# pvphan/camera-calibration

Hardware: AMD Instinct MI355X
Metric: LM iters/sec & residuals/sec, 10k-view checkerboard @1/2/4/8 GPU (higher is better)
Workload: dtype f64

## Files before the change

camera-calibration_amd/_native.py:

```python
import ctypes
import os
import sys

import numpy as np

_HERE = os.path.dirname(os.path.abspath(__file__))
LIB_PATH = os.environ.get("CALIB_LM_LIBRARY") or os.path.join(_HERE, "lib", "libcalib_lm.so")

MODEL_RADTAN, MODEL_FISHEYE = 0, 1
DTYPE_F64, DTYPE_F32 = 0, 1
E_INVALID, E_HIP, E_SINGULAR, E_STATE = -1, -2, -3, -4
TRACE_HEADER = 5
LM_FUSED, LM_TWO_KERNEL = 0, 1

_c_double_p = ctypes.POINTER(ctypes.c_double)
_c_int64_p = ctypes.POINTER(ctypes.c_int64)
_c_int_p = ctypes.POINTER(ctypes.c_int)
_h = ctypes.c_void_p

SIGNATURES = {
    "calib_version": (ctypes.c_int, []),
    "calib_last_error": (ctypes.c_char_p, []),
    "calib_device_count": (ctypes.c_int, [_c_int_p]),
    "calib_create": (ctypes.c_int, [ctypes.c_int, ctypes.c_int, ctypes.c_int, ctypes.POINTER(_h)]),
# ... 17 lines not shown
                                            _c_double_p, ctypes.c_int]),
    "calib_decompose_params": (ctypes.c_int, [ctypes.c_int, ctypes.c_int64, _c_double_p, _c_double_p, _c_double_p,
                                              _c_double_p, ctypes.c_int]),
    "calib_refine_awk": (ctypes.c_int, [_h, _c_double_p, _c_double_p, _c_double_p, ctypes.c_int, ctypes.c_double,
                                        ctypes.c_double, ctypes.c_double, ctypes.c_double, _c_double_p, _c_int_p,
                                        _c_double_p]),
    "calib_lm_begin": (ctypes.c_int, [_h, _c_double_p, ctypes.c_int, ctypes.c_double, ctypes.c_double,
                                      ctypes.c_double, ctypes.c_double]),
    "calib_lm_reduce_size": (ctypes.c_int, [_h, _c_int64_p]),
    "calib_lm_bind_reduce_buffer": (ctypes.c_int, [_h, ctypes.c_void_p]),
    "calib_lm_local": (ctypes.c_int, [_h]),
    "calib_lm_update": (ctypes.c_int, [_h]),
    "calib_lm_run": (ctypes.c_int, [_h, ctypes.c_int, ctypes.c_int]),
    "calib_lm_run_sharded": (ctypes.c_int, [_h, ctypes.c_int, ctypes.c_int]),
    "calib_lm_done": (ctypes.c_int, [_h, _c_int_p]),
    "calib_lm_peek_trace": (ctypes.c_int, [_h, ctypes.c_int, _c_double_p, _c_int_p]),
    "calib_lm_end": (ctypes.c_int, [_h, _c_double_p, _c_double_p, _c_int_p, _c_double_p]),
    "calib_distort_points": (ctypes.c_int, [ctypes.c_int, ctypes.c_int64, _c_double_p, _c_double_p, _c_double_p]),
    "calib_project_with_distortion": (ctypes.c_int, [ctypes.c_int, ctypes.c_int64, _c_double_p, _c_double_p,
                                                     _c_double_p, _c_double_p]),
    "calib_refine_homographies": (ctypes.c_int, [ctypes.c_int64, _c_int64_p, _c_double_p, _c_double_p, _c_double_p,
                                                 ctypes.c_int, ctypes.c_int]),
    "calib_refine_poses": (ctypes.c_int, [ctypes.c_int, ctypes.c_int64, _c_int64_p, _c_double_p, _c_double_p, _c_double_p,
                                          _c_double_p, ctypes.c_int, ctypes.c_double, ctypes.c_double, ctypes.c_double,
                                          ctypes.c_double, _c_double_p, _c_int_p, _c_int_p, ctypes.c_int]),
    "calib_homography_jacobian": (ctypes.c_int, [ctypes.c_int64, _c_double_p, _c_double_p, _c_double_p, ctypes.c_int]),
    "calib_estimate_homographies": (ctypes.c_int, [ctypes.c_int64, _c_int64_p, _c_double_p, _c_double_p, _c_double_p,
                                                   ctypes.c_int, ctypes.c_int]),
    "calib_compute_extrinsics": (ctypes.c_int, [ctypes.c_int64, _c_double_p, _c_double_p, _c_double_p, ctypes.c_int]),
    "calib_distortion_normal_equations": (ctypes.c_int, [ctypes.c_int, ctypes.c_int64, _c_int64_p, _c_double_p,
# ... 94 lines not shown
```

camera-calibration_amd/csrc/calib_lm.hip:

```cpp
#include "../../include/calib_lm.h"
#include "kernels.hpp"
#include "host_rows.hpp"
#include "launch_plan.hpp"

#include <hip/hip_runtime.h>
#include <hip/hip_ext.h>
#include <algorithm>
#include <atomic>
#include <cmath>
#include <cstdio>
#include <cstdlib>
#include <dlfcn.h>
#include <chrono>
#include <future>
#include <memory>
#include <mutex>
#include <thread>
#include <cstring>
#include <new>
#include <string>
#include <type_traits>
#include <vector>

using namespace calib;
// ... 103 lines not shown
    DevBuf<LMState> st, st_eval;
    double* red = nullptr;
    void* comm = nullptr;
    DevBuf<double> rccl_test;
    int comm_ranks = 0, comm_rank = 0;
    void* peer_mem = nullptr;
    std::vector<void*> peer_open;
    DevBuf<unsigned long long*> peer_slots;
    std::vector<unsigned long long*> peer_slot_host;
    DevBuf<int> peer_flags;
    int peer_world = 0, peer_rank = 0;
    unsigned peer_epoch = 0;
    double peer_timeout_s = 60.0;
    bool peer_connected = false;
    bool exchange_round = false;
    int* host_done = nullptr;
    int* host_done_dev = nullptr;
    bool lm_active = false;
    int lm_max_iters = 0;
    int rounds_enqueued = 0;

    bool cov_pending = false;
    std::vector<int64_t> ext_offsets;
    bool ext_offsets_on_device = false;
    DevBuf<int64_t> ext_offsets_dev;
    DevBuf<double> view_err, cov_css, cov_views, cov_cross;
    DevBuf<int> cov_flag;

    bool stage_ready = false;
    void* stage_pinned = nullptr;
// ... 203 lines not shown
StreamMap stream_map(const calib_handle_s* h) {
    StreamMap sm;
    sm.share = h->plan.stream_share;
    sm.n4 = h->uniform_n / 4;
    sm.nv = h->nv;
    return sm;
}
int num_records(const calib_handle_s* h) { return std::max(h->n_items, 1) + h->plan.stream_waves; }

template <int MODEL>
int launch_fused_stream(calib_handle_s* h, const LMState* st, int sel) {
    const LaunchPlan& p = h->plan;
    launch_kind(h, 2, fused_stream_kernel<MODEL>, dim3(p.fused_blocks), dim3(256), 0, (const double*)h->P[0].p, (const double*)h->P[1].p,
                reinterpret_cast<const double2*>(h->uv.p), reinterpret_cast<const double2*>(h->XY.p),
                reinterpret_cast<const double*>(h->Z.p), reinterpret_cast<const double*>(h->VC.p), h->uniform_n,
                h->nv, p.stream_share, (const uint32_t*)h->emit_tab.p, (const int32_t*)h->stream_ops.p, st, sel, h->G[0].p, h->G[1].p,
                h->bpart.p);
    h->n_bpart = p.fused_blocks;
    LAUNCHED(h, "fused_stream_kernel");
    return CALIB_OK;
}

int launch_fused(calib_handle_s* h, const LMState* st, int sel) {
    if (h->plan.fused == FusedForm::Stream)
        return h->model == CALIB_MODEL_RADTAN ? launch_fused_stream<kRadtan>(h, st, sel)
                                              : launch_fused_stream<kFisheye>(h, st, sel);
    if (h->dtype == CALIB_DTYPE_F64)
        return h->model == CALIB_MODEL_RADTAN ? launch_fused_t<kRadtan, double>(h, st, sel)
                                              : launch_fused_t<kFisheye, double>(h, st, sel);
    return h->model == CALIB_MODEL_RADTAN ? launch_fused_t<kRadtan, float>(h, st, sel)
                                          : launch_fused_t<kFisheye, float>(h, st, sel);
// ... 7 lines not shown
    for (int r = 0; r < kPeerInline; ++r) x.slot8[r] = r < (int)h->peer_slot_host.size() ? h->peer_slot_host[(size_t)r] : nullptr;
    x.fault = h->peer_flags.p;
    x.notify = h->host_done_dev;
    x.timeout_ticks = (unsigned long long)(h->peer_timeout_s * 1e8);
    x.epoch = ++h->peer_epoch;
    x.world = h->peer_world;
    x.rank = h->peer_rank;
    return x;
}

int launch_schur(calib_handle_s* h, const LMState* st) {
    const LaunchPlan& p = h->plan;
    dim3 grid(p.schur_blocks, 3);
    auto launch = [&](auto kernel) {
        hipLaunchKernelGGL(kernel, grid, dim3(kSchurBlock), 0, h->stream, h->G[0].p, h->G[1].p, st, view_items(h), h->nv,
                           stream_map(h), h->bpart.p, h->n_bpart, h->part.p);
    };
    auto pick = [&](auto Lc) {
        constexpr int LL = decltype(Lc)::value;
        if (p.stream()) { if (p.wide_heads) launch(schur_kernel<LL, true, true>); else launch(schur_kernel<LL, false, true>); }
        else { if (p.wide_heads) launch(schur_kernel<LL, true, false>); else launch(schur_kernel<LL, false, false>); }
    };
    if (h->L == 10) pick(std::integral_constant<int, 10>{}); else pick(std::integral_constant<int, 9>{});
    LAUNCHED(h, "schur_kernel");
    return CALIB_OK;
}

int launch_schur_reduce(calib_handle_s* h, const LMState* st, double* red) {
    const int VA = variantSize(h->L);
    if (h->nv > 0) {
        const int rc = launch_schur(h, st);
// ... 11 lines not shown

template <int L, typename T>
int launch_update_backsub_t(calib_handle_s* h) {
    const LaunchPlan& p = h->plan;
    UpdArgs<T> a;
    a.G0 = h->G[0].p; a.G1 = h->G[1].p;
    a.st_in = st_cur(h); a.st_out = st_next(h);
    a.red = h->red;
    a.view_item0 = view_items(h);
    a.view_ext = h->view_ext.p;
    a.nv = h->nv;
    a.sm = stream_map(h);
    a.P0 = h->P[0].p; a.P1 = h->P[1].p;
    a.trace = h->trace.p;
    a.VC = reinterpret_cast<T*>(h->VC.p);
    auto launch = [&](auto kernel, int threads, const char* name) -> int {
        hipLaunchKernelGGL(kernel, dim3(p.update_blocks), dim3(threads), 0, h->stream, a);
        LAUNCHED(h, name);
        return CALIB_OK;
    };
    if (p.update == UpdateForm::Small)
        return p.stream() ? launch(update_backsub_small_kernel<L, T, true>, kUpdThreads, "update_backsub_small_kernel")
                          : launch(update_backsub_small_kernel<L, T, false>, kUpdThreads, "update_backsub_small_kernel");
    if (p.update == UpdateForm::Lane)
        return p.stream() ? launch(update_backsub_lane_kernel<L, T, true>, kSchurThreads, "update_backsub_lane_kernel")
                          : launch(update_backsub_lane_kernel<L, T, false>, kSchurThreads, "update_backsub_lane_kernel");
    return p.stream() ? launch(update_backsub_kernel<L, T, true>, kSchurThreads, "update_backsub_kernel")
                      : launch(update_backsub_kernel<L, T, false>, kSchurThreads, "update_backsub_kernel");
}

// ... 512 lines not shown
    }
    if (h->host_done) {
        if (h->lm_active) SYNC_H(h);
        *h->host_done = 0;
        s.notify = h->host_done_dev;
    }
    s.cur = 1;
    s.fixed_mask = (int)h->fixed_mask;
    s.max_iters = max_iters;
    HIP_TRY(hipMemsetAsync(h->st.p, 0, 2 * sizeof(LMState), h->stream));
    HIP_TRY(hipMemcpyAsync(h->st.p, &s, sizeof(s), hipMemcpyHostToDevice, h->stream));
    SYNC_H(h);
    h->lm_active = true;
    h->lm_max_iters = max_iters;
    h->rounds_enqueued = 0;
    return CALIB_OK;
}

int calib_lm_local(calib_handle_t h) {
    CHECK_H(h);
    if (!h->lm_active) return fail(CALIB_E_STATE, "calib_lm_begin has not been called");
    LMState* st = st_cur(h);
    int rc = CALIB_OK;
    if (h->rounds_enqueued == 0) {
        rc = launch_view_setup_any(h, h->P[0].p, h->P[1].p, st, 1);
        if (rc) return rc;
    }
    if (h->lm_mode == CALIB_LM_FUSED) {
        rc = launch_fused(h, st, 1);
        if (rc) return rc;
// ... 2 lines not shown
    h->n_bpart = 0;
    for (const auto& c : h->chunks) {
        rc = launch_jacobian(h, h->P[0].p, h->P[1].p, st, 1, true, true, false, false, c.p0, c.p1);
        if (rc) return rc;
        rc = launch_gram(h, st, 1, c.item0, c.item1, c.p0);
        if (rc) return rc;
    }
    return launch_schur_reduce(h, st, h->red);
}

int calib_lm_update(calib_handle_t h) {
    CHECK_H(h);
    if (!h->lm_active) return fail(CALIB_E_STATE, "calib_lm_begin has not been called");
    const int rc = launch_update_backsub(h);
    h->rounds_enqueued += 1;
    return rc;
}

namespace {
int peer_fault_check(calib_handle_s* h) {
    if (!h->peer_connected) return CALIB_OK;
    int fault = 0;
    HIP_TRY(hipMemcpy(&fault, h->peer_flags.p, sizeof(int), hipMemcpyDeviceToHost));
    if (fault)
        return fail(CALIB_E_HIP, "peer exchange: a rank's contribution did not arrive before the deadline "
                                 "(the ranks no longer run in lockstep, or a peer died)");
    return CALIB_OK;
}
}

int calib_lm_done(calib_handle_t h, int* out_done) {
    CHECK_H(h);
    if (!h->lm_active || !out_done) return fail(CALIB_E_STATE, "no LM run active");
    LMState s;
    HIP_TRY(hipMemcpyAsync(&s, st_cur(h), sizeof(s), hipMemcpyDeviceToHost, h->stream));
    SYNC_H(h);
    *out_done = s.done;
    return peer_fault_check(h);
}

int calib_lm_peek_trace(calib_handle_t h, int iter, double* out_row, int* out_iters) {
    CHECK_H(h);
    if (!h->lm_active || !out_row || !out_iters) return fail(CALIB_E_STATE, "no LM run active");
    if (iter < 0 || iter >= h->lm_max_iters) return fail(CALIB_E_INVALID, "trace row out of range");
    LMState s;
    const size_t w = (size_t)(CALIB_TRACE_HEADER + h->L);
    HIP_TRY(hipMemcpyAsync(&s, st_cur(h), sizeof(s), hipMemcpyDeviceToHost, h->stream));
    HIP_TRY(hipMemcpyAsync(out_row, h->trace.p + (size_t)iter * w, w * 8, hipMemcpyDeviceToHost, h->stream));
    SYNC_H(h);
    *out_iters = s.iters;
    return CALIB_OK;
}

namespace {
int lm_run(calib_handle_t h, int rounds, int check_every, bool sharded);
}

int calib_lm_run(calib_handle_t h, int rounds, int check_every) { return lm_run(h, rounds, check_every, false); }

int calib_lm_run_sharded(calib_handle_t h, int rounds, int check_every) {
    if (h && !h->comm && !h->peer_connected)
        return fail(CALIB_E_STATE, "neither calib_peer_connect nor calib_rccl_init has been called");
    return lm_run(h, rounds, check_every, true);
}

namespace {
int lm_run(calib_handle_t h, int rounds, int check_every, bool sharded) {
    CHECK_H(h);
    if (!h->lm_active) return fail(CALIB_E_STATE, "calib_lm_begin has not been called");
    const bool peers = sharded && h->peer_connected;
    for (int i = 0; i < rounds; ++i) {
        h->exchange_round = peers;
        int rc = calib_lm_local(h);
        h->exchange_round = false;
        if (rc) return rc;
        if (sharded && !peers) {
            rc = calib_lm_allreduce(h);
            if (rc) return rc;
        }
        rc = calib_lm_update(h);
        if (rc) return rc;
        if (peers && h->host_done && *static_cast<volatile int*>(h->host_done) == 2)
            return fail(CALIB_E_HIP, "peer exchange: a rank's contribution did not arrive before the deadline "
                                     "(the ranks no longer run in lockstep, or a peer died); no further rounds are enqueued");
        if (check_every > 0 && !sharded && h->host_done) {
            if (*static_cast<volatile int*>(h->host_done)) break;
        } else if (check_every > 0 && (i + 1) % check_every == 0 && i + 1 < rounds) {
            int done = 0;
            rc = calib_lm_done(h, &done);
            if (rc) return rc;
            if (done) break;
        }
    }
    return CALIB_OK;
}
}

int calib_rccl_load(const char* librccl_path) {
    std::lock_guard<std::mutex> lock(g_rccl_mutex);
    if (g_rccl.lib) return CALIB_OK;
    if (!librccl_path) return fail(CALIB_E_INVALID, "librccl path is null");
    void* lib = dlopen(librccl_path, RTLD_NOW | RTLD_GLOBAL);
    if (!lib) return fail(CALIB_E_HIP, std::string("dlopen librccl: ") + dlerror());
    RcclApi a;
    a.lib = lib;
    a.getUniqueId = reinterpret_cast<decltype(a.getUniqueId)>(dlsym(lib, "ncclGetUniqueId"));
    a.commInitRank = reinterpret_cast<decltype(a.commInitRank)>(dlsym(lib, "ncclCommInitRank"));
    a.allReduce = reinterpret_cast<decltype(a.allReduce)>(dlsym(lib, "ncclAllReduce"));
// ... 861 lines not shown
```

camera-calibration_amd/csrc/kernels.hpp:

```cpp
#pragma once
#include "point_model.hpp"
#include <stdint.h>
#include <type_traits>

namespace calib {

constexpr int kTile = 256;
constexpr int kGramChunk = 512;
constexpr int kGramUnroll = 4;
constexpr int kGRows = 0;
constexpr int kGStride = 96;
__host__ __device__ __forceinline__ constexpr int gvSlot(int L, int j) { return j < 5 ? L + 1 + j : 16 + L + 2; }
__host__ __device__ __forceinline__ constexpr int gvOfSlot(int L, int slot) {
    const int m = slot >> 4, n = (slot & 15) - L;
    return (m == 0 && n >= 1 && n <= 5) ? n - 1 : ((m == 1 && n == 2) ? 5 : -1);
}
constexpr int kPartStride = 112;
constexpr int kMaxL = 10;

constexpr int kEmitZero = 256;
constexpr int kEmitTile = 264;
constexpr int kEmitTabSize = kGStride + kPartStride;
inline void buildEmitTable(int C, uint32_t* tab ) {
    const int L = C - 6;
// ... 49 lines not shown
    o.x = __builtin_bit_cast(float, __builtin_amdgcn_ds_bpermute(a, __builtin_bit_cast(int, v.x)));
    o.y = __builtin_bit_cast(float, __builtin_amdgcn_ds_bpermute(a, __builtin_bit_cast(int, v.y)));
    return o;
}

struct LMState {
    double lam, err_cur, last_err, lam_min, lam_max, err_min;
    int cur;
    int round;
    int iters;
    int max_iters;
    int done;
    int error;
    int accepted_last;
    int fixed_mask;
    int* notify;
    double dc[kMaxL];
    double B[kMaxL * kMaxL];
    double gc[kMaxL];
};

__host__ __device__ constexpr int variantSize(int L) { return 2 * L * L + 2 * L + 2; }
__host__ __device__ constexpr int reduceSize(int L) { return 2 * variantSize(L); }

__device__ __forceinline__ const double* selectP(const double* P0, const double* P1,
                                                 const LMState* st, int sel) {
    if (sel == 0) return P0;
    return (st->cur ^ 1) ? P1 : P0;
}

// ... 240 lines not shown

struct BlockAcc {
    double d0u = 0.0, d0v = 0.0, d1u = 0.0, d1v = 0.0, d2u = 0.0;
    int bi, bj, trow, tcol0, tcol1, tcol2;
    __device__ __forceinline__ explicit BlockAcc(int lane) {
        const int k = lane >> 4;
        bi = (lane >> 2) & 3; bj = lane & 3;
        trow = 4 * bi + k; tcol0 = 4 * bi + bj; tcol1 = 4 * ((bi + 1) & 3) + bj; tcol2 = 4 * ((bi + 2) & 3) + bj;
    }
    __device__ __forceinline__ void contract(const double2& ja, const double2& jb, double ha, double hc) {
        d0u = __builtin_amdgcn_mfma_f64_4x4x4f64(ja.x, ja.x, d0u, 0, 0, 0);
        d0v = __builtin_amdgcn_mfma_f64_4x4x4f64(ja.y, ja.y, d0v, 0, 0, 0);
        d1u = __builtin_amdgcn_mfma_f64_4x4x4f64(ja.x, jb.x, d1u, 0, 0, 0);
        d1v = __builtin_amdgcn_mfma_f64_4x4x4f64(ja.y, jb.y, d1v, 0, 0, 0);
        d2u = __builtin_amdgcn_mfma_f64_4x4x4f64(ha, hc, d2u, 0, 0, 0);
    }
    __device__ __forceinline__ void park(double* TU, double* TV) const {
        TU[trow * 16 + tcol0] = d0u;  TV[trow * 16 + tcol0] = d0v;
        TU[trow * 16 + tcol1] = d1u;  TV[trow * 16 + tcol1] = d1v;
        TU[tcol1 * 16 + trow] = d1u;  TV[tcol1 * 16 + trow] = d1v;
        double* T2nd = bi < 2 ? TU : TV;
        T2nd[trow * 16 + tcol2] = d2u;
        T2nd[tcol2 * 16 + trow] = d2u;
    }
};

template <int MODEL, typename T, bool G44, bool MULTI>
__global__ __launch_bounds__(64 * kFusedWaves, (sizeof(T) == 4 ? (MULTI ? 5 : 6)
                                                             : (ModelTraits<MODEL>::C == 16 ? 4 : 3))) void fused_kernel(const double* __restrict__ P0, const double* __restrict__ P1,
                                                    const typename Pair<T>::type* __restrict__ uv,
// ... 267 lines not shown
            const Src sv = locate(iv, true);
            put(sv.lane, sv.acc == 1 ? 7 : (sv.acc == 3 ? 9 : 10), 1, slot);
        }
    }
    return ok;
}

constexpr int kStreamMinBlocks = 4;
template <int MODEL>
__global__ __launch_bounds__(64 * kFusedWaves, kStreamMinBlocks) void fused_stream_kernel(const double* __restrict__ P0, const double* __restrict__ P1,
                                                              const double2* __restrict__ uv, const double2* __restrict__ XY,
                                                              const double* __restrict__ Z, const double* __restrict__ VC,
                                                              int n, int nv, int share,
                                                              const uint32_t* __restrict__ emit_tab,
                                                              const int32_t* __restrict__ stream_ops,
                                                              const LMState* __restrict__ st, int sel,
                                                              double* __restrict__ G0, double* __restrict__ G1,
                                                              double* __restrict__ part) {
    using T = double;
    using T2 = double2;
    constexpr int C = ModelTraits<MODEL>::C, L = C - 6;
    using Slab = FusedSlab<T, C>;
    constexpr int ROWS = Slab::ROWS, WAVES = Slab::WAVES, SLAB = Slab::SIZE;
    constexpr bool RCOL = Slab::RCOL, ONES = Slab::ONES;
    __shared__ __attribute__((aligned(16))) unsigned char smem[Slab::BYTES];
    __shared__ __attribute__((aligned(16))) double svc[WAVES][2 * kViewStride];
    __shared__ __attribute__((aligned(16))) int32_t sops[64 * kStreamOps];
    int fin = 0, useP1 = 0;
    auto readState = [&]() {
        if (sel) {
            fin = st->done;
            useP1 = st->cur ^ 1;
        }
    };
    const int lane = threadIdx.x & 63;
    const int wave = __builtin_amdgcn_readfirstlane(threadIdx.x >> 6);
    const int k = lane >> 4;
    const int sl = Slab::pointOf(lane);
    T2* slab = reinterpret_cast<T2*>(smem) + wave * SLAB;
    BlockAcc blk(lane);
    double* Gbase = G0;
    auto ofView = [](int i) { return i >= L && i < L + 6; };
    const bool keep0 = !(ofView(blk.trow) || ofView(blk.tcol0)), keep1 = !(ofView(blk.trow) || ofView(blk.tcol1)),
               keep2 = !(ofView(blk.trow) || ofView(blk.tcol2));
    {
        const int4* src = reinterpret_cast<const int4*>(stream_ops) + 3 * lane;
        int4* dst = reinterpret_cast<int4*>(sops) + 3 * lane;
// ... 62 lines not shown
            const T* s = VC + (int64_t)__builtin_amdgcn_readfirstlane(view) * kViewStride;
#pragma unroll
            for (int i = 0; i < kViewStride - 1; ++i) vcs[i] = s[i];
        };
        bool strad = straddles(p0, vend);
        if (strad) vc_n = stagedLoad(va); else scalarLoad(va);
        readState();
        if (fin) return;
        if (useP1) sp = spB;
        Gbase = useP1 ? G1 : G0;
        const T2* src = slab + Slab::rowOff(k);
        const int c = lane & 15, c1 = (c + 4) & 15, c2 = (c + 8) & 15, jh = (lane >> 3) & 1;
        const T* h0 = reinterpret_cast<const T*>(src + c) + jh;
        const T* h2 = reinterpret_cast<const T*>(src + c2) + jh;
        PointState<MODEL, T> pst;
        for (int q0 = p0; q0 < p1; q0 += 64) {
            const int qe = q0 + 64 < p1 ? q0 + 64 : p1;
            const int q = q0 + sl;
            const T2 m = m_n, xy = xy_n;
            const T z = z_n;
            const double vcx = vc_n;
            const bool more = q0 + 64 < p1;
            const bool passes = vend < qe;
            const int ve2 = passes ? vend + n : vend, va2 = passes ? va + 1 : va;
            const bool strad2 = more && straddles(q0 + 64, ve2);
            const int vfirst2 = ve2 <= q0 + 64 ? va2 + 1 : va2;
            if (more) {
                pn = q + 64 < p1 ? q + 64 : p1 - 1;
                m_n = uv[pn]; xy_n = XY[pn]; z_n = Z[pn];
                if (strad2) vc_n = stagedLoad(va2);
// ... 18 lines not shown
                }
                __builtin_amdgcn_wave_barrier();
                jacobian_point<MODEL, T>(sp, vcl, xy.x, xy.y, z, u, v, Jc);
            }
            T2 res;
            res.x = m.x - u;
            res.y = m.y - v;
            if (more && !strad2) scalarLoad(vfirst2);
            strad = strad2;
            constexpr int NCH = C - 5 + 1;
            T2 ch[NCH];
#pragma unroll
            for (int i = 0; i < C - 5; ++i) ch[i] = Jc[5 + i];
            ch[NCH - 1] = res;
            auto colOf = [](int i) { return i < C - 5 ? 5 + i : (RCOL ? 15 : 4); };
#pragma unroll
            for (int i = 0; i + 1 < NCH; i += 2) {
                unsigned a[4], b[4];
                __builtin_memcpy(a, &ch[i], sizeof(T2));
                __builtin_memcpy(b, &ch[i + 1], sizeof(T2));
#pragma unroll
                for (int d = 0; d < 4; ++d) {
                    const auto r = __builtin_amdgcn_permlane32_swap(a[d], b[d], false, false);
                    a[d] = r[0];
                    b[d] = r[1];
                }
                __builtin_memcpy(&ch[i], a, sizeof(T2));
                __builtin_memcpy(&ch[i + 1], b, sizeof(T2));
            }
#pragma unroll
            for (int half = 0; half < 2; ++half) {
                const int ps = q0 + ROWS * half;
                if (ps >= p1) break;
                __builtin_amdgcn_wave_barrier();
                T2* row = slab + Slab::rowOff(sl & (ROWS - 1));
                if ((lane >> 5) == half) {
                    T* rh = reinterpret_cast<T*>(row);
                    rh[0] = Jc[0].x; rh[3] = Jc[1].y; rh[4] = Jc[2].x;
                }
#pragma unroll
                for (int i = 0; i + 1 < NCH; i += 2) row[lane < 32 ? colOf(i) : colOf(i + 1)] = ch[i + half];
                if ((NCH & 1) && (lane >> 5) == half) row[colOf(NCH - 1)] = ch[NCH - 1];
                __builtin_amdgcn_wave_barrier();
                const int ng = (p1 - ps >= ROWS ? ROWS : p1 - ps) >> 2;
                const int jb = (vend - ps) >> 2;
                auto runFixed = [&](auto FROMc, auto TOc) {
                    constexpr int FROM = decltype(FROMc)::value, TO = decltype(TOc)::value;
                    if constexpr (FROM < TO) {
                        T2 ja = src[66 * FROM + c], jbb = src[66 * FROM + c1];
                        double ha = h0[2 * 66 * FROM], hc = h2[2 * 66 * FROM];
#pragma unroll
                        for (int s = FROM; s < TO; ++s) {
                            T2 na = ja, nb = jbb;
                            double nha = ha, nhc = hc;
                            if (s + 1 < TO) {
                                na = src[66 * (s + 1) + c]; nb = src[66 * (s + 1) + c1];
                                nha = h0[2 * 66 * (s + 1)]; nhc = h2[2 * 66 * (s + 1)];
                            }
                            __builtin_amdgcn_sched_barrier(0);
                            blk.contract(ja, jbb, ha, hc);
                            __builtin_amdgcn_sched_barrier(0);
                            ja = na; jbb = nb; ha = nha; hc = nhc;
                        }
                    }
                };
                auto nextView = [&]() {
                    emitView(slot);
                    va += 1;
                    vend += n;
                    slot = va;
                };
                constexpr int NG = ROWS / 4;
                using std::integral_constant;
                if (ng == NG && jb >= NG) {
                    runFixed(integral_constant<int, 0>{}, integral_constant<int, NG>{});
                } else if (ng == NG) {
                    auto boundaryAt = [&](auto JBc) {
                        constexpr int JB = decltype(JBc)::value;
                        runFixed(integral_constant<int, 0>{}, integral_constant<int, JB>{});
                        nextView();
                        runFixed(integral_constant<int, JB>{}, integral_constant<int, NG>{});
                    };
                    switch (jb) {
                    case 0: boundaryAt(integral_constant<int, 0>{}); break;
                    case 1: boundaryAt(integral_constant<int, 1>{}); break;
                    case 2: boundaryAt(integral_constant<int, 2>{}); break;
                    case 3: boundaryAt(integral_constant<int, 3>{}); break;
                    case 4: boundaryAt(integral_constant<int, 4>{}); break;
                    case 5: boundaryAt(integral_constant<int, 5>{}); break;
                    case 6: boundaryAt(integral_constant<int, 6>{}); break;
                    default: boundaryAt(integral_constant<int, 7>{}); break;
                    }
                } else {
                    const int sb = jb < ng ? jb : ng;
                    auto runGroups = [&](int from, int to) {
                        switch (from) {
#define CALIB_GROUP_CASE(S) case S: if (to <= S) break; blk.contract(src[66 * S + c], src[66 * S + c1], h0[2 * 66 * S], h2[2 * 66 * S]); [[fallthrough]];
                        CALIB_GROUP_CASE(0) CALIB_GROUP_CASE(1) CALIB_GROUP_CASE(2) CALIB_GROUP_CASE(3)
                        CALIB_GROUP_CASE(4) CALIB_GROUP_CASE(5) CALIB_GROUP_CASE(6) CALIB_GROUP_CASE(7)
#undef CALIB_GROUP_CASE
                        default: break;
                        }
                    };
                    runGroups(0, sb);
                    if (jb < ng) {
                        nextView();
                        runGroups(sb, ng);
                    }
                }
            }
        }
        emitView(slot);
    } else {
        readState();
        if (fin) return;
    }
    {
        double* TU = Slab::tileU(slab);
        double* TV = Slab::tileV(slab);
        __builtin_amdgcn_wave_barrier();
        blk.park(TU, TV);
        if (lane == 0) { TU[kEmitZero] = 0.0; TV[kEmitZero] = 0.0; }
    }
    __syncthreads();
    Slab::writePartial(smem, emit_tab, part);
}

// ... 174 lines not shown
        t.x = (T)o18[2 * j];
        t.y = (T)o18[2 * j + 1];
        reinterpret_cast<T2*>(dst)[j] = t;
    }
}

constexpr int kSchurBlock = 256;
constexpr int kSchurViewsPerBlock = kSchurBlock / 16;

template <int L, bool WIDE, bool STREAM>
__global__ __launch_bounds__(kSchurBlock, (!WIDE && STREAM) ? 3 : 4) void schur_kernel(const double* __restrict__ G0,
                                                            const double* __restrict__ G1,
                                                            const LMState* __restrict__ st,
                                                            const int* __restrict__ view_item0,
                                                            int nv, StreamMap sm, const double* __restrict__ bpart,
                                                            int n_bpart, double* __restrict__ part) {
    constexpr int VA = variantSize(L);
    constexpr int kNfail = 2 * L * L + 2 * L, kSse = kNfail + 1;
    __shared__ double sfail[kSchurViewsPerBlock];
    __shared__ double stile[kSchurBlock / 64][256];
    const int tid = threadIdx.x, lane = tid & 63, wave = tid >> 6, c = tid & 15, grp = tid >> 4, k = lane >> 4;

    if (blockIdx.y == 2) {
        constexpr int NF = L * L + L + 1;
        double* out = part + (int64_t)blockIdx.x * VA;
        const int t = tid & 127, half = tid >> 7;
        double s0 = 0.0, s1 = 0.0, s2 = 0.0, s3 = 0.0;
        if (t < NF) {
            const int64_t step = (int64_t)gridDim.x * 2;
            int64_t it = (int64_t)blockIdx.x * 2 + half;
            const double* src = bpart + t;
// ... 12 lines not shown
        if (tid < NF) {
            const double tot = sh[tid] + sh[128 + tid];
            out[tid < L * L ? tid : (tid < L * L + L ? 2 * L * L + (tid - L * L) : kSse)] = tot;
        }
        return;
    }

    const double* G = blockIdx.y ? G1 : G0;
    double V[21], b[6];
    int v0 = blockIdx.x * kSchurViewsPerBlock;
    if (v0 + grp < nv) load_view_head<L, WIDE>(G, view_span<STREAM>(view_item0, sm, v0 + grp), c, V, b);
    if (st->done) return;
    const bool boot = st->round == 0;
    const int cand = st->cur ^ 1;
    const int variant = (int)blockIdx.y == cand ? 0 : 1;
    double* out = part + ((int64_t)variant * gridDim.x + blockIdx.x) * VA;
    if (variant == 1 && boot) {
        for (int i = tid; i < VA; i += kSchurBlock) out[i] = 0.0;
        return;
    }
    const double lam = variant == 0 ? (boot ? st->lam : st->lam / 10) : st->lam * 10;

    d4 acc = {0.0, 0.0, 0.0, 0.0};
    double nfail = 0.0;
    const int stride = gridDim.x * kSchurViewsPerBlock;
    while (v0 < nv) {
        double z[6];
#pragma unroll
        for (int m = 0; m < 6; ++m) z[m] = 0.0;
        const bool live = v0 + grp < nv;
// ... 269 lines not shown
    }
    return ok;
}

struct LMDecision { int cur; double lam; bool acc; };
__device__ __forceinline__ LMDecision lm_decide(int cur, double lam, int round, double err_cand, double err_cur) {
    if (round == 0) return {cur ^ 1, lam, false};
    if (err_cand < err_cur) return {cur ^ 1, lam / 10, true};
    return {cur, lam * 10, false};
}

template <int L>
__device__ __forceinline__ bool lm_update_step(const LMState* __restrict__ in, LMState* __restrict__ out,
                                               const double* __restrict__ red, double* __restrict__ P0,
                                               double* __restrict__ P1, double* __restrict__ trace,
                                               bool writer, int i, int& cur_out, double& lam_out,
                                               double (&dc)[L]) {
    constexpr int VA = variantSize(L);
    constexpr int kNfail = 2 * L * L + 2 * L, kSse = kNfail + 1;
    const bool w0 = writer && i == 0;
    double* Pb[2] = {P0, P1};
    int cur = in->cur;
    const int round = in->round;
    const double err_cand = red[kSse];
    double lam = in->lam;
    double sA[L], sB[L], bA[L], bS[L];
    double rhsA = 0.0, rhsB = 0.0, gA = 0.0, gS = 0.0;
#pragma unroll
    for (int j = 0; j < L; ++j) { sA[j] = 0.0; sB[j] = 0.0; bA[j] = 0.0; bS[j] = 0.0; }
    if (i < L) {
#pragma unroll
// ... 8 lines not shown
        gA = red[2 * L * L + i];
        gS = in->gc[i];
    }
    const double nfailA = red[kNfail], nfailB = red[VA + kNfail];
    if (in->done) {
        if (writer) for (int j = i; j < (int)(sizeof(LMState) / 8); j += 16)
            reinterpret_cast<double*>(out)[j] = reinterpret_cast<const double*>(in)[j];
        return false;
    }
    bool useB = false;
    bool done = false;
    double err_cur_new = err_cand, last_err = err_cand;
    int iters = in->iters, accepted = 0;
    const double err_cur = in->err_cur;
    const LMDecision dec = lm_decide(cur, lam, round, err_cand, err_cur);
    if (round > 0) {
        const int it = round - 1;
        if (trace && writer) {
            double* row = trace + (int64_t)it * (5 + L);
            if (i < L) row[5 + i] = Pb[cur][i];
            if (i == 0) { row[0] = it; row[1] = err_cur; row[2] = err_cand; row[3] = lam; row[4] = dec.acc ? 1.0 : 0.0; }
        }
        useB = !dec.acc;
        done = !(in->lam_min < dec.lam && dec.lam < in->lam_max) || err_cur < in->err_min || it + 1 >= in->max_iters;
        last_err = err_cur;
        err_cur_new = dec.acc ? err_cand : err_cur;
        iters = it + 1;
        accepted = dec.acc ? 1 : 0;
    }
    cur = dec.cur;
    lam = dec.lam;
    int error = 0;
    if (!done && (useB ? nfailB : nfailA) > 0.0) { error = -3; done = true; }

    double row[L + 1], brow[L];
    const double gci = useB ? gS : gA;
#pragma unroll
    for (int j = 0; j < L; ++j) {
        brow[j] = useB ? bS[j] : bA[j];
        row[j] = brow[j] - (useB ? sB[j] : sA[j]);
    }
    row[L] = gci - (useB ? rhsB : rhsA);
#pragma unroll
// ... 28 lines not shown
        if (i < L) {
#pragma unroll
            for (int j = 0; j < L; ++j) out->B[i * L + j] = brow[j];
            out->gc[i] = gci;
            double dci = 0.0;
#pragma unroll
            for (int c = 0; c < L; ++c) if (c == i) dci = dc[c];
            out->dc[i] = dci;
            if (!done) Pb[cur ^ 1][i] = fixed_i ? Pb[cur][i] : Pb[cur][i] + dci;
        }
        if (w0) {
            out->lam = lam; out->err_cur = err_cur_new; out->last_err = last_err;
            out->lam_min = in->lam_min; out->lam_max = in->lam_max; out->err_min = in->err_min;
            out->cur = cur; out->round = round + 1; out->iters = iters; out->max_iters = in->max_iters;
            out->done = done ? 1 : 0; out->error = error; out->accepted_last = accepted; out->fixed_mask = fixed_mask;
            out->notify = in->notify;
            if (done && in->notify) __hip_atomic_store(in->notify, 1, __ATOMIC_RELAXED, __HIP_MEMORY_SCOPE_SYSTEM);
        }
    }
    cur_out = cur;
    lam_out = lam;
    return !done;
}

template <int L, typename T>
__device__ __forceinline__ void finish_view(const double (&V)[21], const double (&invd)[6], const double (&z)[6],
                                            double coef, int c, int v, const int* __restrict__ view_ext,
                                            const double* __restrict__ Pc, double* __restrict__ Pn,
                                            T* __restrict__ VC) {
    double w[6];
// ... 35 lines not shown
    if (c < 2) dst[16 + c] = (T)(c == 0 ? o18[16] : o18[17]);
}

template <typename T>
struct UpdArgs {
    const double* G0; const double* G1;
    const LMState* st_in; LMState* st_out;
    const double* red;
    const int* view_item0;
    const int* view_ext;
    int nv;
    StreamMap sm;
    double* P0; double* P1;
    double* trace;
    T* VC;
};

template <int L, typename T>
__device__ __forceinline__ void decide_and_publish(const UpdArgs<T>& a, int c, double (&sdec)[L + 3]) {
    const bool writer = blockIdx.x == 0;
    int cur = 0;
    double lam = 0.0, dc[L];
    const bool go = lm_update_step<L>(a.st_in, a.st_out, a.red, a.P0, a.P1, a.trace, writer, c, cur, lam, dc);
    if (c == 0) { sdec[0] = go ? 1.0 : 0.0; sdec[1] = (double)cur; sdec[2] = lam; }
    if (c < L) {
        double dci = 0.0;
#pragma unroll
        for (int j = 0; j < L; ++j) if (j == c) dci = dc[j];
        sdec[3 + c] = dci;
    }
}

template <int L, typename T, bool STREAM>
__global__ __launch_bounds__(kSchurThreads, 4) void update_backsub_kernel(UpdArgs<T> a) {
    const int tid = threadIdx.x, c = tid & 15;
    __shared__ double sdec[L + 3];
    if (tid < 16) decide_and_publish<L>(a, c, sdec);
    __syncthreads();
// ... 748 lines not shown
```

camera-calibration_amd/csrc/launch_plan.hpp:

```cpp
#pragma once
#include "../../include/calib_lm.h"
#include "kernels.hpp"

#include <algorithm>
#include <cstdint>
#include <cstdlib>
#include <cstring>

namespace calib {

constexpr int kUpdSmallViews = 4096;
constexpr int kUpdLaneViews = 24576;
constexpr int kWideHeadViews = 4096;

struct Knobs {
    int lm_mode = CALIB_LM_FUSED;
    int head_loads = 0;
    int items_per_wave = 0;
    int upd_lane_views = kUpdLaneViews;
    int upd_small_views = kUpdSmallViews;
    int gram_form = 0;
    int stream_mode = -1;
    int stream_waves = 0;
    int gram_wpi = 0;
    int64_t chunk_points = (int64_t)1 << 26;
    bool timing = false;
};

inline Knobs readKnobs() {
    Knobs k;
    if (const char* e = std::getenv("CALIB_LM_MODE")) k.lm_mode = std::atoi(e) ? CALIB_LM_TWO_KERNEL : CALIB_LM_FUSED;
    if (const char* e = std::getenv("CALIB_HEAD_LOADS")) k.head_loads = std::strcmp(e, "narrow") == 0 ? 1 : (std::strcmp(e, "wide") == 0 ? 2 : 0);
    if (const char* e = std::getenv("CALIB_ITEMS_PER_WAVE")) k.items_per_wave = std::max(0, std::min(16, std::atoi(e)));
    if (const char* e = std::getenv("CALIB_UPD_LANE_VIEWS")) k.upd_lane_views = std::max(1, std::atoi(e));
    if (const char* e = std::getenv("CALIB_UPD_SMALL_VIEWS")) k.upd_small_views = std::max(0, std::atoi(e));
    if (const char* e = std::getenv("CALIB_GRAM_FORM")) k.gram_form = std::strcmp(e, "tile") == 0 ? 1 : (std::strcmp(e, "block") == 0 ? 2 : 0);
    if (const char* e = std::getenv("CALIB_FUSED_STREAM")) k.stream_mode = std::atoi(e) > 0 ? 1 : (std::atoi(e) == 0 ? 0 : -1);
    if (const char* e = std::getenv("CALIB_STREAM_WAVES")) k.stream_waves = std::max(0, std::atoi(e));
    if (const char* e = std::getenv("CALIB_GRAM_WPI")) {
        const int w = std::atoi(e);
        if (w == 1 || w == 2 || w == 4) k.gram_wpi = w;
    }
    if (const char* e = std::getenv("CALIB_CHUNK_POINTS")) k.chunk_points = std::max<int64_t>(1, std::atoll(e));
    k.timing = std::getenv("CALIB_TIMING") != nullptr;
    return k;
}

struct ShardShape {
    int nv = 0, n_items = 0, uniform_n = 0;
    int64_t MN = 0;
};

enum class FusedForm {
    TwoKernel,
    Tile,
    TileMulti,
    Block44,
    Stream,
// ... 6 lines not shown

struct LaunchPlan {
    FusedForm fused = FusedForm::Tile;
    int fused_wpi = 1;
    int ipw = 1;
    int fused_blocks = 0;
    int gram_wpi = 1;
    int stream_share = 0;
    int stream_waves = 0;
    bool wide_heads = false;
    UpdateForm update = UpdateForm::Small;
    int schur_blocks = 1;
    int update_blocks = 1;
    bool stream() const { return stream_share > 0; }
};

inline LaunchPlan makePlan(const ShardShape& s, int dtype, int lm_mode, const Knobs& k, int num_cus) {
    LaunchPlan p;
    const double avg = s.n_items ? (double)s.MN / s.n_items : 0.0;
    p.gram_wpi = avg >= 128 ? 4 : (avg >= 64 ? 2 : 1);
    p.fused_wpi = s.n_items >= 2048 ? 1 : p.gram_wpi;
    if (k.gram_wpi > 0) p.gram_wpi = p.fused_wpi = k.gram_wpi;

    const int un = s.uniform_n;
    const bool can = dtype == CALIB_DTYPE_F64 && un >= 64 && (un & 3) == 0 && s.MN < ((int64_t)1 << 31) && s.nv >= 1;
    if (lm_mode == CALIB_LM_FUSED && can && k.stream_mode != 0) {
        const int slots = k.stream_waves > 0 ? k.stream_waves : kFusedWaves * kStreamMinBlocks * num_cus;
        const int waves = std::max(1, std::min(slots, s.nv));
        if (k.stream_mode == 1 || s.nv >= 2 * slots) {
            const int64_t groups = (int64_t)s.nv * (un / 4);
// ... 41 lines not shown
```

camera-calibration_amd/engine.py:

```python
import ctypes

import numpy as np

from . import _native as nat
from . import fixed as fixedmod

LAMBDA_INITIAL = 1e-3
LAMBDA_MIN = 1e-10
LAMBDA_MAX = 1e+10
PT_ERROR_MIN = 1e-12

MODEL_IDS = {"radtan": nat.MODEL_RADTAN, "fisheye": nat.MODEL_FISHEYE}
NUM_SHARED = {nat.MODEL_RADTAN: 10, nat.MODEL_FISHEYE: 9}
DTYPE_IDS = {"f64": nat.DTYPE_F64, "fp64": nat.DTYPE_F64, "float64": nat.DTYPE_F64,
             "f32": nat.DTYPE_F32, "fp32": nat.DTYPE_F32, "float32": nat.DTYPE_F32}


def _stack(arrays, width):
    M = len(arrays)
    if M == 0:
        return np.zeros(0, dtype=np.int64), np.empty((0, width))
    fast = True
    for a in arrays:
        if type(a) is not np.ndarray or a.dtype != np.float64 or a.ndim != 2 or a.shape[1] != width:
# ... 288 lines not shown
        nat.check(self._lib.calib_rccl_selftest(self._h, float(timeoutSeconds)))

    def rcclShutdown(self):
        nat.check(self._lib.calib_rccl_shutdown(self._h))

    def lmAllReduce(self):
        nat.check(self._lib.calib_lm_allreduce(self._h))

    def synchronize(self):
        nat.check(self._lib.calib_synchronize(self._h))

    def lmDone(self):
        d = ctypes.c_int(0)
        nat.check(self._lib.calib_lm_done(self._h, ctypes.byref(d)))
        return bool(d.value)

    def peekTrace(self, it):
        row = np.zeros(nat.TRACE_HEADER + self.L)
        n = ctypes.c_int(0)
        nat.check(self._lib.calib_lm_peek_trace(self._h, int(it), nat.dptr(row), ctypes.byref(n)))
        return row, n.value

    def lmEnd(self):
        P = np.empty(self.K)
        trace = np.zeros((max(self._lmMaxIters, 1), nat.TRACE_HEADER + self.L))
        sse = ctypes.c_double(0.0)
        iters = ctypes.c_int(0)
        nat.check(self._lib.calib_lm_end(self._h, nat.dptr(P), ctypes.byref(sse), ctypes.byref(iters),
                                         nat.dptr(trace)))
        return sse.value, P, iters.value, trace[:iters.value]
# ... 256 lines not shown
```

include/calib_lm.h:

```cpp
#ifndef CALIB_LM_H
#define CALIB_LM_H

#include <stdint.h>

#ifdef __cplusplus
extern "C" {
#endif

typedef struct calib_handle_s* calib_handle_t;

enum { CALIB_MODEL_RADTAN = 0, CALIB_MODEL_FISHEYE = 1 };
enum { CALIB_DTYPE_F64 = 0, CALIB_DTYPE_F32 = 1 };
enum {
    CALIB_OK = 0,
    CALIB_E_INVALID = -1,
    CALIB_E_HIP = -2,
    CALIB_E_SINGULAR = -3,
    CALIB_E_STATE = -4
};

#define CALIB_TRACE_HEADER 5

int         calib_version(void);
const char* calib_last_error(void);
// ... 35 lines not shown
int calib_compose_params(int model, int64_t num_views, const double* A, const double* W, const double* k,
                         double* P_out, int device_id);
int calib_decompose_params(int model, int64_t num_views, const double* P, double* A_out, double* W_out,
                           double* k_out, int device_id);
int calib_refine_awk(calib_handle_t h, double* A_inout, double* W_inout, double* k_inout, int max_iters,
                     double lam_init, double lam_min, double lam_max, double err_min,
                     double* out_sse, int* out_iters, double* out_trace);

int calib_lm_begin(calib_handle_t h, const double* P0, int max_iters,
                   double lam_init, double lam_min, double lam_max, double err_min);
int calib_lm_reduce_size(calib_handle_t h, int64_t* out_num_doubles);
int calib_lm_bind_reduce_buffer(calib_handle_t h, void* reduce_dev);
int calib_lm_local(calib_handle_t h);
int calib_lm_update(calib_handle_t h);
int calib_lm_run(calib_handle_t h, int rounds, int check_every);
int calib_lm_run_sharded(calib_handle_t h, int rounds, int check_every);

#define CALIB_PEER_HANDLE_BYTES 64
int calib_peer_prepare(calib_handle_t h, int nranks, int rank, void* out_handle64);
int calib_peer_connect(calib_handle_t h, const void* handles, double timeout_s);
int calib_peer_selftest(calib_handle_t h, int rounds, double timeout_s);
int calib_peer_shutdown(calib_handle_t h);

int calib_rccl_load(const char* librccl_path);
int calib_rccl_unique_id(void* out_id128);
int calib_rccl_init(calib_handle_t h, int nranks, int rank, const void* id128);
int calib_rccl_init_deadline(calib_handle_t h, int nranks, int rank, const void* id128, double timeout_s);
int calib_rccl_selftest(calib_handle_t h, double timeout_s);
int calib_rccl_shutdown(calib_handle_t h);
int calib_lm_allreduce(calib_handle_t h);
// ... 45 lines not shown
```

Baseline: 31.10 billion.

## Add cheap probe rounds after repeated LM rejections in stream mode

After a configurable number of consecutive rejected LM steps, the next round runs as a probe. It computes only the residual and diagonal contractions, skips view emission and the candidate Schur variant, and replays the round if the cheap evaluation says the step would be accepted. The host loop re-enqueues rounds until the target count of decided rounds is reached, which adds a blocking state readback per batch. This is meant to avoid full normal-equation assembly on rounds that usually get rejected, at the cost of redoing a round when the probe accepts plus extra host syncs.

```diff
diff --git a/camera-calibration_amd/_native.py b/camera-calibration_amd/_native.py
--- a/camera-calibration_amd/_native.py
+++ b/camera-calibration_amd/_native.py
@@ -55,6 +55,7 @@
     "calib_lm_run": (ctypes.c_int, [_h, ctypes.c_int, ctypes.c_int]),
     "calib_lm_run_sharded": (ctypes.c_int, [_h, ctypes.c_int, ctypes.c_int]),
     "calib_lm_done": (ctypes.c_int, [_h, _c_int_p]),
+    "calib_lm_probe_stats": (ctypes.c_int, [_h, _c_int_p, _c_int_p]),
     "calib_lm_peek_trace": (ctypes.c_int, [_h, ctypes.c_int, _c_double_p, _c_int_p]),
     "calib_lm_end": (ctypes.c_int, [_h, _c_double_p, _c_double_p, _c_int_p, _c_double_p]),
     "calib_distort_points": (ctypes.c_int, [ctypes.c_int, ctypes.c_int64, _c_double_p, _c_double_p, _c_double_p]),
diff --git a/camera-calibration_amd/csrc/calib_lm.hip b/camera-calibration_amd/csrc/calib_lm.hip
--- a/camera-calibration_amd/csrc/calib_lm.hip
+++ b/camera-calibration_amd/csrc/calib_lm.hip
@@ -141,6 +141,8 @@
     double peer_timeout_s = 60.0;
     bool peer_connected = false;
     bool exchange_round = false;
+    int probe_round = 0;
+    int rounds_decided = 0;
     int* host_done = nullptr;
     int* host_done_dev = nullptr;
     bool lm_active = false;
@@ -374,7 +376,7 @@
     launch_kind(h, 2, fused_stream_kernel<MODEL>, dim3(p.fused_blocks), dim3(256), 0, (const double*)h->P[0].p, (const double*)h->P[1].p,
                 reinterpret_cast<const double2*>(h->uv.p), reinterpret_cast<const double2*>(h->XY.p),
                 reinterpret_cast<const double*>(h->Z.p), reinterpret_cast<const double*>(h->VC.p), h->uniform_n,
-                h->nv, p.stream_share, (const uint32_t*)h->emit_tab.p, (const int32_t*)h->stream_ops.p, st, sel, h->G[0].p, h->G[1].p,
+                h->nv, p.stream_share, (const uint32_t*)h->emit_tab.p, (const int32_t*)h->stream_ops.p, st, sel, h->probe_round > 0 ? 1 : 0, h->G[0].p, h->G[1].p,
                 h->bpart.p);
     h->n_bpart = p.fused_blocks;
     LAUNCHED(h, "fused_stream_kernel");
@@ -412,7 +414,7 @@
     dim3 grid(p.schur_blocks, 3);
     auto launch = [&](auto kernel) {
         hipLaunchKernelGGL(kernel, grid, dim3(kSchurBlock), 0, h->stream, h->G[0].p, h->G[1].p, st, view_items(h), h->nv,
-                           stream_map(h), h->bpart.p, h->n_bpart, h->part.p);
+                           stream_map(h), h->bpart.p, h->n_bpart, h->part.p, h->probe_round > 0 ? 1 : 0);
     };
     auto pick = [&](auto Lc) {
         constexpr int LL = decltype(Lc)::value;
@@ -454,6 +456,7 @@
     a.P0 = h->P[0].p; a.P1 = h->P[1].p;
     a.trace = h->trace.p;
     a.VC = reinterpret_cast<T*>(h->VC.p);
+    a.probe_after = h->probe_round;
     auto launch = [&](auto kernel, int threads, const char* name) -> int {
         hipLaunchKernelGGL(kernel, dim3(p.update_blocks), dim3(threads), 0, h->stream, a);
         LAUNCHED(h, name);
@@ -996,6 +999,7 @@
     h->lm_active = true;
     h->lm_max_iters = max_iters;
     h->rounds_enqueued = 0;
+    h->rounds_decided = 0;
     return CALIB_OK;
 }
 
@@ -1028,6 +1032,7 @@
     if (!h->lm_active) return fail(CALIB_E_STATE, "calib_lm_begin has not been called");
     const int rc = launch_update_backsub(h);
     h->rounds_enqueued += 1;
+    if (h->probe_round == 0) h->rounds_decided += 1;
     return rc;
 }
 
@@ -1053,6 +1058,17 @@
     return peer_fault_check(h);
 }
 
+int calib_lm_probe_stats(calib_handle_t h, int* out_probe_rounds, int* out_redone_rounds) {
+    CHECK_H(h);
+    if (!h->st.p) return fail(CALIB_E_STATE, "calib_lm_begin has not been called");
+    LMState s;
+    HIP_TRY(hipMemcpyAsync(&s, st_cur(h), sizeof(s), hipMemcpyDeviceToHost, h->stream));
+    SYNC_H(h);
+    if (out_probe_rounds) *out_probe_rounds = s.n_probe;
+    if (out_redone_rounds) *out_redone_rounds = s.n_redo;
+    return CALIB_OK;
+}
+
 int calib_lm_peek_trace(calib_handle_t h, int iter, double* out_row, int* out_iters) {
     CHECK_H(h);
     if (!h->lm_active || !out_row || !out_iters) return fail(CALIB_E_STATE, "no LM run active");
@@ -1083,29 +1099,40 @@
     CHECK_H(h);
     if (!h->lm_active) return fail(CALIB_E_STATE, "calib_lm_begin has not been called");
     const bool peers = sharded && h->peer_connected;
-    for (int i = 0; i < rounds; ++i) {
-        h->exchange_round = peers;
-        int rc = calib_lm_local(h);
-        h->exchange_round = false;
-        if (rc) return rc;
-        if (sharded && !peers) {
-            rc = calib_lm_allreduce(h);
+    const int probe = sharded ? 0 : probeAfter(h->plan, h->knobs);
+    const int target = h->rounds_decided + rounds;
+    bool over = false;
+    for (int todo = rounds; todo > 0 && !over;) {
+        for (int i = 0; i < todo; ++i) {
+            h->exchange_round = peers;
+            h->probe_round = probe;
+            int rc = calib_lm_local(h);
+            h->exchange_round = false;
+            if (!rc && sharded && !peers) rc = calib_lm_allreduce(h);
+            if (!rc) rc = calib_lm_update(h);
+            h->probe_round = 0;
             if (rc) return rc;
-        }
-        rc = calib_lm_update(h);
-        if (rc) return rc;
-        if (peers && h->host_done && *static_cast<volatile int*>(h->host_done) == 2)
-            return fail(CALIB_E_HIP, "peer exchange: a rank's contribution did not arrive before the deadline "
-                                     "(the ranks no longer run in lockstep, or a peer died); no further rounds are enqueued");
-        if (check_every > 0 && !sharded && h->host_done) {
-            if (*static_cast<volatile int*>(h->host_done)) break;
-        } else if (check_every > 0 && (i + 1) % check_every == 0 && i + 1 < rounds) {
-            int done = 0;
-            rc = calib_lm_done(h, &done);
-            if (rc) return rc;
-            if (done) break;
-        }
-    }
+            if (peers && h->host_done && *static_cast<volatile int*>(h->host_done) == 2)
+                return fail(CALIB_E_HIP, "peer exchange: a rank's contribution did not arrive before the deadline "
+                                         "(the ranks no longer run in lockstep, or a peer died); no further rounds are enqueued");
+            if (check_every > 0 && !sharded && h->host_done) {
+                if (*static_cast<volatile int*>(h->host_done)) { over = true; break; }
+            } else if (check_every > 0 && (i + 1) % check_every == 0 && i + 1 < todo) {
+                int done = 0;
+                rc = calib_lm_done(h, &done);
+                if (rc) return rc;
+                if (done) { over = true; break; }
+            }
+        }
+        todo = 0;
+        if (probe > 0 && !over) {
+            LMState s;
+            HIP_TRY(hipMemcpyAsync(&s, st_cur(h), sizeof(s), hipMemcpyDeviceToHost, h->stream));
+            SYNC_H(h);
+            if (!s.done && s.round < target) todo = target - s.round;
+        }
+    }
+    if (probe > 0) h->rounds_decided = target;
     return CALIB_OK;
 }
 }
diff --git a/camera-calibration_amd/csrc/kernels.hpp b/camera-calibration_amd/csrc/kernels.hpp
--- a/camera-calibration_amd/csrc/kernels.hpp
+++ b/camera-calibration_amd/csrc/kernels.hpp
@@ -1,5 +1,6 @@
 #pragma once
 #include "point_model.hpp"
+#include <stddef.h>
 #include <stdint.h>
 #include <type_traits>
 
@@ -87,6 +88,10 @@
     int error;
     int accepted_last;
     int fixed_mask;
+    int probe;
+    int rej;
+    int n_probe;
+    int n_redo;
     int* notify;
     double dc[kMaxL];
     double B[kMaxL * kMaxL];
@@ -357,6 +362,10 @@
         d1u = __builtin_amdgcn_mfma_f64_4x4x4f64(ja.x, jb.x, d1u, 0, 0, 0);
         d1v = __builtin_amdgcn_mfma_f64_4x4x4f64(ja.y, jb.y, d1v, 0, 0, 0);
         d2u = __builtin_amdgcn_mfma_f64_4x4x4f64(ha, hc, d2u, 0, 0, 0);
+    }
+    __device__ __forceinline__ void contractDiag(const double2& ja) {
+        d0u = __builtin_amdgcn_mfma_f64_4x4x4f64(ja.x, ja.x, d0u, 0, 0, 0);
+        d0v = __builtin_amdgcn_mfma_f64_4x4x4f64(ja.y, ja.y, d0v, 0, 0, 0);
     }
     __device__ __forceinline__ void park(double* TU, double* TV) const {
         TU[trow * 16 + tcol0] = d0u;  TV[trow * 16 + tcol0] = d0v;
@@ -654,7 +663,7 @@
                                                               int n, int nv, int share,
                                                               const uint32_t* __restrict__ emit_tab,
                                                               const int32_t* __restrict__ stream_ops,
-                                                              const LMState* __restrict__ st, int sel,
+                                                              const LMState* __restrict__ st, int sel, int probe_ok,
                                                               double* __restrict__ G0, double* __restrict__ G1,
                                                               double* __restrict__ part) {
     using T = double;
@@ -666,11 +675,12 @@
     __shared__ __attribute__((aligned(16))) unsigned char smem[Slab::BYTES];
     __shared__ __attribute__((aligned(16))) double svc[WAVES][2 * kViewStride];
     __shared__ __attribute__((aligned(16))) int32_t sops[64 * kStreamOps];
-    int fin = 0, useP1 = 0;
+    int fin = 0, useP1 = 0, probe = 0;
     auto readState = [&]() {
         if (sel) {
             fin = st->done;
             useP1 = st->cur ^ 1;
+            if (probe_ok) probe = __builtin_amdgcn_readfirstlane(st->probe);
         }
     };
     const int lane = threadIdx.x & 63;
@@ -763,6 +773,14 @@
         const T* h0 = reinterpret_cast<const T*>(src + c) + jh;
         const T* h2 = reinterpret_cast<const T*>(src + c2) + jh;
         PointState<MODEL, T> pst;
+        auto runShare = [&](auto PROBEc) {
+        constexpr bool PROBE = decltype(PROBEc)::value;
+        if constexpr (PROBE) {
+            T2 zero;
+            zero.x = 0.0; zero.y = 0.0;
+            __builtin_amdgcn_wave_barrier();
+            for (int i = lane; i < SLAB; i += 64) slab[i] = zero;
+        }
         for (int q0 = p0; q0 < p1; q0 += 64) {
             const int qe = q0 + 64 < p1 ? q0 + 64 : p1;
             const int q = q0 + sl;
@@ -811,6 +829,7 @@
             for (int i = 0; i < C - 5; ++i) ch[i] = Jc[5 + i];
             ch[NCH - 1] = res;
             auto colOf = [](int i) { return i < C - 5 ? 5 + i : (RCOL ? 15 : 4); };
+            if constexpr (!PROBE) {
 #pragma unroll
             for (int i = 0; i + 1 < NCH; i += 2) {
                 unsigned a[4], b[4];
@@ -825,12 +844,16 @@
                 __builtin_memcpy(&ch[i], a, sizeof(T2));
                 __builtin_memcpy(&ch[i + 1], b, sizeof(T2));
             }
+            }
 #pragma unroll
             for (int half = 0; half < 2; ++half) {
                 const int ps = q0 + ROWS * half;
                 if (ps >= p1) break;
                 __builtin_amdgcn_wave_barrier();
                 T2* row = slab + Slab::rowOff(sl & (ROWS - 1));
+                if constexpr (PROBE) {
+                    if ((lane >> 5) == half) row[colOf(NCH - 1)] = res;
+                } else {
                 if ((lane >> 5) == half) {
                     T* rh = reinterpret_cast<T*>(row);
                     rh[0] = Jc[0].x; rh[3] = Jc[1].y; rh[4] = Jc[2].x;
@@ -838,12 +861,19 @@
 #pragma unroll
                 for (int i = 0; i + 1 < NCH; i += 2) row[lane < 32 ? colOf(i) : colOf(i + 1)] = ch[i + half];
                 if ((NCH & 1) && (lane >> 5) == half) row[colOf(NCH - 1)] = ch[NCH - 1];
+                }
                 __builtin_amdgcn_wave_barrier();
                 const int ng = (p1 - ps >= ROWS ? ROWS : p1 - ps) >> 2;
                 const int jb = (vend - ps) >> 2;
                 auto runFixed = [&](auto FROMc, auto TOc) {
                     constexpr int FROM = decltype(FROMc)::value, TO = decltype(TOc)::value;
-                    if constexpr (FROM < TO) {
+                    if constexpr (PROBE) {
+                        T2 ja[TO > FROM ? TO - FROM : 1];
+#pragma unroll
+                        for (int s = FROM; s < TO; ++s) ja[s - FROM] = src[66 * s + c];
+#pragma unroll
+                        for (int s = FROM; s < TO; ++s) blk.contractDiag(ja[s - FROM]);
+                    } else if constexpr (FROM < TO) {
                         T2 ja = src[66 * FROM + c], jbb = src[66 * FROM + c1];
                         double ha = h0[2 * 66 * FROM], hc = h2[2 * 66 * FROM];
 #pragma unroll
@@ -862,7 +892,7 @@
                     }
                 };
                 auto nextView = [&]() {
-                    emitView(slot);
+                    if constexpr (!PROBE) emitView(slot);
                     va += 1;
                     vend += n;
                     slot = va;
@@ -892,7 +922,10 @@
                     const int sb = jb < ng ? jb : ng;
                     auto runGroups = [&](int from, int to) {
                         switch (from) {
-#define CALIB_GROUP_CASE(S) case S: if (to <= S) break; blk.contract(src[66 * S + c], src[66 * S + c1], h0[2 * 66 * S], h2[2 * 66 * S]); [[fallthrough]];
+#define CALIB_GROUP_CASE(S) case S: if (to <= S) break; \
+                            if constexpr (PROBE) blk.contractDiag(src[66 * S + c]); \
+                            else blk.contract(src[66 * S + c], src[66 * S + c1], h0[2 * 66 * S], h2[2 * 66 * S]); \
+                            [[fallthrough]];
                         CALIB_GROUP_CASE(0) CALIB_GROUP_CASE(1) CALIB_GROUP_CASE(2) CALIB_GROUP_CASE(3)
                         CALIB_GROUP_CASE(4) CALIB_GROUP_CASE(5) CALIB_GROUP_CASE(6) CALIB_GROUP_CASE(7)
 #undef CALIB_GROUP_CASE
@@ -907,7 +940,9 @@
                 }
             }
         }
-        emitView(slot);
+        if constexpr (!PROBE) emitView(slot);
+        };
+        if (probe) runShare(std::true_type{}); else runShare(std::false_type{});
     } else {
         readState();
         if (fin) return;
@@ -1112,7 +1147,7 @@
                                                             const LMState* __restrict__ st,
                                                             const int* __restrict__ view_item0,
                                                             int nv, StreamMap sm, const double* __restrict__ bpart,
-                                                            int n_bpart, double* __restrict__ part) {
+                                                            int n_bpart, double* __restrict__ part, int probe_ok) {
     constexpr int VA = variantSize(L);
     constexpr int kNfail = 2 * L * L + 2 * L, kSse = kNfail + 1;
     __shared__ double sfail[kSchurViewsPerBlock];
@@ -1155,6 +1190,7 @@
     const bool boot = st->round == 0;
     const int cand = st->cur ^ 1;
     const int variant = (int)blockIdx.y == cand ? 0 : 1;
+    if (variant == 0 && probe_ok && st->probe) return;
     double* out = part + ((int64_t)variant * gridDim.x + blockIdx.x) * VA;
     if (variant == 1 && boot) {
         for (int i = tid; i < VA; i += kSchurBlock) out[i] = 0.0;
@@ -1454,7 +1490,7 @@
 __device__ __forceinline__ bool lm_update_step(const LMState* __restrict__ in, LMState* __restrict__ out,
                                                const double* __restrict__ red, double* __restrict__ P0,
                                                double* __restrict__ P1, double* __restrict__ trace,
-                                               bool writer, int i, int& cur_out, double& lam_out,
+                                               bool writer, int i, int probe_after, int& cur_out, double& lam_out,
                                                double (&dc)[L]) {
     constexpr int VA = variantSize(L);
     constexpr int kNfail = 2 * L * L + 2 * L, kSse = kNfail + 1;
@@ -1493,6 +1529,20 @@
     int iters = in->iters, accepted = 0;
     const double err_cur = in->err_cur;
     const LMDecision dec = lm_decide(cur, lam, round, err_cand, err_cur);
+    const bool probe = probe_after > 0 && in->probe != 0;
+    static_assert(offsetof(LMState, probe) % 8 == 0 && offsetof(LMState, rej) == offsetof(LMState, probe) + 4 &&
+                  offsetof(LMState, n_redo) == offsetof(LMState, n_probe) + 4 && offsetof(LMState, n_probe) % 8 == 0,
+                  "the patched words of an undecided round");
+    if (probe && dec.acc) {
+        if (writer) for (int j = i; j < (int)(sizeof(LMState) / 8); j += 16) {
+            double w = reinterpret_cast<const double*>(in)[j];
+            if (j == (int)(offsetof(LMState, probe) / 8)) w = __hiloint2double(in->rej, 0);
+            if (j == (int)(offsetof(LMState, n_probe) / 8)) w = __hiloint2double(in->n_redo + 1, in->n_probe + 1);
+            reinterpret_cast<double*>(out)[j] = w;
+        }
+        return false;
+    }
+    int rej = 0;
     if (round > 0) {
         const int it = round - 1;
         if (trace && writer) {
@@ -1506,6 +1556,7 @@
         err_cur_new = dec.acc ? err_cand : err_cur;
         iters = it + 1;
         accepted = dec.acc ? 1 : 0;
+        rej = dec.acc ? 0 : in->rej + 1;
     }
     cur = dec.cur;
     lam = dec.lam;
@@ -1564,6 +1615,8 @@
             out->lam_min = in->lam_min; out->lam_max = in->lam_max; out->err_min = in->err_min;
             out->cur = cur; out->round = round + 1; out->iters = iters; out->max_iters = in->max_iters;
             out->done = done ? 1 : 0; out->error = error; out->accepted_last = accepted; out->fixed_mask = fixed_mask;
+            out->probe = (probe_after > 0 && !done && rej >= probe_after) ? 1 : 0; out->rej = rej;
+            out->n_probe = in->n_probe + (probe ? 1 : 0); out->n_redo = in->n_redo;
             out->notify = in->notify;
             if (done && in->notify) __hip_atomic_store(in->notify, 1, __ATOMIC_RELAXED, __HIP_MEMORY_SCOPE_SYSTEM);
         }
@@ -1629,6 +1682,7 @@
     double* P0; double* P1;
     double* trace;
     T* VC;
+    int probe_after;
 };
 
 template <int L, typename T>
@@ -1636,7 +1690,7 @@
     const bool writer = blockIdx.x == 0;
     int cur = 0;
     double lam = 0.0, dc[L];
-    const bool go = lm_update_step<L>(a.st_in, a.st_out, a.red, a.P0, a.P1, a.trace, writer, c, cur, lam, dc);
+    const bool go = lm_update_step<L>(a.st_in, a.st_out, a.red, a.P0, a.P1, a.trace, writer, c, a.probe_after, cur, lam, dc);
     if (c == 0) { sdec[0] = go ? 1.0 : 0.0; sdec[1] = (double)cur; sdec[2] = lam; }
     if (c < L) {
         double dci = 0.0;
diff --git a/camera-calibration_amd/csrc/launch_plan.hpp b/camera-calibration_amd/csrc/launch_plan.hpp
--- a/camera-calibration_amd/csrc/launch_plan.hpp
+++ b/camera-calibration_amd/csrc/launch_plan.hpp
@@ -24,6 +24,8 @@
     int stream_waves = 0;
     int gram_wpi = 0;
     int64_t chunk_points = (int64_t)1 << 26;
+    int probe_mode = 1;
+    int probe_after = 2;
     bool timing = false;
 };
 
@@ -42,6 +44,12 @@
         if (w == 1 || w == 2 || w == 4) k.gram_wpi = w;
     }
     if (const char* e = std::getenv("CALIB_CHUNK_POINTS")) k.chunk_points = std::max<int64_t>(1, std::atoll(e));
+    if (const char* e = std::getenv("CALIB_LM_PROBE")) {
+        if (std::strcmp(e, "force") == 0) k.probe_mode = 2;
+        else if (std::strcmp(e, "0") == 0) k.probe_mode = 0;
+        else if (std::strcmp(e, "1") == 0) k.probe_mode = 1;
+    }
+    if (const char* e = std::getenv("CALIB_LM_PROBE_AFTER")) k.probe_after = std::max(1, std::atoi(e));
     k.timing = std::getenv("CALIB_TIMING") != nullptr;
     return k;
 }
@@ -78,6 +86,11 @@
     int update_blocks = 1;
     bool stream() const { return stream_share > 0; }
 };
+
+inline int probeAfter(const LaunchPlan& p, const Knobs& k) {
+    if (k.probe_mode == 0) return 0;
+    return (p.fused == FusedForm::Stream || k.probe_mode == 2) ? k.probe_after : 0;
+}
 
 inline LaunchPlan makePlan(const ShardShape& s, int dtype, int lm_mode, const Knobs& k, int num_cus) {
     LaunchPlan p;
diff --git a/camera-calibration_amd/engine.py b/camera-calibration_amd/engine.py
--- a/camera-calibration_amd/engine.py
+++ b/camera-calibration_amd/engine.py
@@ -326,6 +326,11 @@
         d = ctypes.c_int(0)
         nat.check(self._lib.calib_lm_done(self._h, ctypes.byref(d)))
         return bool(d.value)
+
+    def lmProbeStats(self):
+        p, r = ctypes.c_int(0), ctypes.c_int(0)
+        nat.check(self._lib.calib_lm_probe_stats(self._h, ctypes.byref(p), ctypes.byref(r)))
+        return p.value, r.value
 
     def peekTrace(self, it):
         row = np.zeros(nat.TRACE_HEADER + self.L)
diff --git a/include/calib_lm.h b/include/calib_lm.h
--- a/include/calib_lm.h
+++ b/include/calib_lm.h
@@ -73,6 +73,7 @@
 int calib_lm_local(calib_handle_t h);
 int calib_lm_update(calib_handle_t h);
 int calib_lm_run(calib_handle_t h, int rounds, int check_every);
+int calib_lm_probe_stats(calib_handle_t h, int* out_probe_rounds, int* out_redone_rounds);
 int calib_lm_run_sharded(calib_handle_t h, int rounds, int check_every);
 
 #define CALIB_PEER_HANDLE_BYTES 64
```

New measurement: 41.53 billion (median of 6 runs). 33.6% higher.
